# jbrea/BayesianOptimization.jl

Measured on AMD Instinct MI355X. Metric: acquisition-candidates/sec (N=3000,d=8), higher is better.
Workload: dtype f64

## Files before the change

bayesianoptimization.jl_amd/csrc/bohip.hip:

```cpp
#include "../../include/bohip.h"
#include "../../include/bohip_paths.h"
#include "../../include/bohip_fit.h"
#include "../../include/bohip_qei.h"
#include "../../include/bohip_acq.h"
#include "kernels_linalg.hip"
#include "kernels_chol.hip"
#include "kernels_exec.hip"
#include "kernels_score.hip"
#include "kernels_batch.hip"
#include "kernels_sample.hip"
#include "kernels_qei.hip"
#include "kernels_path.hip"
#include "kernels_ascent.hip"
#include "kernels_fit.hip"
#include "kernels_small.hip"
#include "direct_l.h"

#include <algorithm>
#include <atomic>
#include <chrono>
#include <cerrno>
#include <cmath>
#include <cstdio>
#include <cstring>
// ... 36 lines not shown
struct bohip_gp {
    int device = 0, d = 0, kern = 0;
    int64_t n = 0, cap = 0, ld = 0;
    double *dX = nullptr, *dy = nullptr, *dL = nullptr, *dW = nullptr, *dWT = nullptr, *dS = nullptr;
    double *dalpha = nullptr, *dr = nullptr, *dt = nullptr, *dmll = nullptr;
    double* dApp = nullptr;
    int* dinfo = nullptr;
    unsigned* dchol_flags = nullptr;
    double* dchol_idl = nullptr;
    std::vector<double> hX, hy;
    double loglen[DMAX], logsig = 0.0, lognoise = -2.0, beta = 0.0;
    bool stale = true;
    int64_t n_factored = 0;
    hipStream_t stream = nullptr, own_stream = nullptr;
    hipStream_t side_stream = nullptr;
    hipEvent_t ev_panels = nullptr, ev_bulk = nullptr;
    hipStream_t col_stream = nullptr;
    hipEvent_t ev_inv = nullptr;
    hipEvent_t ev_gate = nullptr;
    ExTask* dex_tasks = nullptr;
    size_t ex_cap = 0;
    bool ex_bulk4_ok = false;
    int ex_T = 0, ex_nsf = 0, ex_inv_g = -1, ex_grp_min = -1, ex_qbeg[EX_NQ + 1] = {0};
    bool w_done = false;
    double* dKsT = nullptr;
    unsigned long long* dclk = nullptr;
    int* dpieces = nullptr;
    std::vector<int> hpieces;
    int n_pieces = 0, pieces_T = -1;
    int64_t pieces_cap = 0;
    int64_t pieces_alpha = -1;
    int64_t kst_rows = 0;
    int64_t chunk_now = 0;
    int64_t score_launches = 0;
    double *dVT = nullptr, *dUT = nullptr;
    int64_t vt_rows = 0;
    double *dq = nullptr, *dmu_raw = nullptr, *dXs = nullptr, *dmu = nullptr, *dvar = nullptr, *dscore = nullptr;
    int64_t q_cap = 0, r_cap = 0, xs_cap = 0;
    Best *dblock_best = nullptr, *dbest = nullptr;
    int64_t bb_cap = 0;
    unsigned* dfz_cnt = nullptr;
    Best* dfz_best = nullptr;
    int64_t fz_cap = 0;
    bool fz_dirty = false;
    char* dpr = nullptr;
    size_t pr_bytes = 0;
    std::vector<int> hpr_pieces;
    int* pr_pieces_at = nullptr;
    unsigned* hprune_stat = nullptr;
    unsigned prune_seen = 0;
    bool prune_retry = false;
    int prune_r2_form = -1;
    int prune_skip = 0;
    double* dBV = nullptr;
    int64_t bv_rows = 0, bv_ld = 0;
    char* dbatch = nullptr;
    size_t batch_bytes = 0;
    double* dgrad = nullptr;
    double asc_ftol_abs = 0.0, asc_xtol_rel = 0.0, asc_stopval = INFINITY;
    double asc_maxtime = 0.0;
    int64_t batch_hint = 0;
    double* dsplit = nullptr;
    int64_t split_cap = 0;
    const SmallFold* asc_fold = nullptr;
    bool asc_fold_done = false;
    const unsigned* asc_go = nullptr;
    double* dgparts = nullptr;
    unsigned* dgcount = nullptr;
    double* dsm = nullptr;
    size_t sm_bytes = 0;
    unsigned* dsm_cnt = nullptr;
    int sm_cnt_T = 0;
    double* hpin = nullptr;
    double* dschur = nullptr;
    AscentState asc{};
    double* asc_block = nullptr;
    int* asc_ints = nullptr;
    double* asc_hio = nullptr;
    double* asc_dio = nullptr;
    size_t asc_io_cap = 0;
    int* asc_hints = nullptr;
    double* asc_bounds = nullptr;
    Best* asc_best = nullptr;
    int64_t asc_cap = 0;
    int64_t grad_cap = 0;
    Best* dthompson = nullptr;
    double* ddmll_parts = nullptr;
    double* fit_ws = nullptr;
    char* fit_io = nullptr;
    size_t fit_ws_bytes = 0, fit_io_bytes = 0;
    double *dVV = nullptr, *dcov = nullptr;
    int64_t cov_cap = 0;
    double *sjL = nullptr, *sjS = nullptr, *sjW = nullptr, *sjWT = nullptr, *sjF = nullptr, *sj_scal = nullptr;
    int* sj_info = nullptr;
    Best* sj_part = nullptr;
    int64_t sj_cap = 0;
    size_t sjF_cap = 0, sj_part_cap = 0;
    char* qei_ws = nullptr;
    size_t qei_bytes = 0;
    int64_t dmll_cap = 0;
    int64_t thompson_cap = 0;
    void* comm = nullptr;
    int comm_rank = 0, comm_n = 0;
    int64_t comm_exchanges = 0;
    Best *csend = nullptr, *crecv = nullptr, *cfinal = nullptr;
    int64_t crec_cap = 0;
// ... 122 lines not shown
    {
        const size_t Tm = (size_t)(g->ld / TILE) + 1;
        HIPCHK(hipMalloc(&g->dchol_flags, chol_flag_words((int)std::min<size_t>(Tm, CHOL_DF_TCAP)) * sizeof(unsigned)));
        HIPCHK(hipMalloc(&g->dchol_idl, Tm * CH_PANELS * 256 * 8));
    }
    HIPCHK(hipMemsetAsync(g->dL, 0, mat, g->stream));
    HIPCHK(hipMemsetAsync(g->dW, 0, mat, g->stream));
    HIPCHK(hipMemsetAsync(g->dWT, 0, mat, g->stream));
    HIPCHK(hipMemsetAsync(g->dS, 0, mat, g->stream));
    if (g->n > 0) {
        HIPCHK(hipMemcpyAsync(g->dX, g->hX.data(), (size_t)g->n * g->d * 8, hipMemcpyHostToDevice, g->stream));
        HIPCHK(hipMemcpyAsync(g->dy, g->hy.data(), (size_t)g->n * 8, hipMemcpyHostToDevice, g->stream));
    }
    g->stale = true;
    return 0;
}

static int g_bulk_pieces = 4;
static int g_sample_mfma_min = 200;
static int g_path_mfma_min = 24;
static int g_split = 1;
static int g_asc_wg_nmax = 256;
static const double g_asc_first_step = 0.1;
static int g_asc_fold = 1;
static int g_asc_lockstep = 0;
static int g_small_mfma = 1;
static int g_small_m = 0;
static int g_small_r = -1;
static int g_inv_hi_h = 16;
static int g_chol_df = 1;
static bool g_chol_df_strict = false;
static bool g_chol_df_dump = false;
static int g_chol_df_tmax = 96;
static std::atomic<int> g_chol_df_skip{0}, g_chol_df_backoff{0};
static unsigned long long g_chol_spin_ticks = CH_SPIN_TICKS_DEFAULT;
static int g_chol_exec_patience_us = 1000;
static int g_chol_exec_fill_inv = 1;
static int g_chol_exec_inv_pairs = 0;
static std::atomic<int> g_chol_inv_grp_min{28};
static std::atomic<int> g_chol_inv_g{8};
static int g_chol_nsf = 3;
static int g_chol_exec_urgent = -1;
static int g_chol_exec_second = 1;
static int g_small_zero_copy = 1;
static int g_chol_exec_nbu = 2;
static int g_chol_exec_fast = -1;
static int g_chol_exec_pairs = -1;
static int g_chol_exec_wgs = -1;
static int g_append_alpha_inc = 1;
static int g_fuse_finish = 1;
static int64_t g_chunk_rows_forced = 0;
static int g_halve_lo = -1, g_halve_hi = -1;
static int g_prune_m = -1;
static int g_ks8 = 1;
static int launch_gemm_nt(bohip_gp* g, const GemmNTParams& p, int batch = 1, hipStream_t st = nullptr, bool hi = false) {
    if (p.mt <= 0 || p.nt64 <= 0 || p.kc <= 0 || batch <= 0) return 0;
    if (hi) hipLaunchKernelGGL(k_gemm_nt_hi, dim3(p.mt * p.nt64, batch), dim3(GEMM_THREADS_8), glds3_lds_bytes<4>(), st ? st : g->stream, p);
    else hipLaunchKernelGGL(k_gemm_nt, dim3(p.mt * p.nt64, batch), dim3(GEMM_THREADS_8), glds3_lds_bytes<4>(), st ? st : g->stream, p);
    HIPCHK(hipGetLastError());
    return 0;
}

static int device_cus();
static void read_dev_knobs() {
#if BOHIP_DEV_KNOBS
    struct Knob { const char* name; int* v; int lo, hi; };
    static int chunk_rows = 0, dump = 0;
    const Knob knobs[] = {
        {"BOHIP_CHOL_DF_TMAX", &g_chol_df_tmax, 0, CHOL_DF_TCAP}, {"BOHIP_INV_HI_H", &g_inv_hi_h, 0, 1 << 20},
        {"BOHIP_CHOL_EXEC_PAIRS", &g_chol_exec_pairs, -1, 64},
        {"BOHIP_CHOL_EXEC_URGENT", &g_chol_exec_urgent, 1, 1 << 20}, {"BOHIP_CHOL_NSF", &g_chol_nsf, 1, CH_NSF_MAX},
        {"BOHIP_CHOL_EXEC_PATIENCE_US", &g_chol_exec_patience_us, 0, 1 << 30}, {"BOHIP_CHOL_EXEC_FILL_INV", &g_chol_exec_fill_inv, 0, 1},
        {"BOHIP_CHOL_EXEC_INV_PAIRS", &g_chol_exec_inv_pairs, 0, 1}, {"BOHIP_CHOL_EXEC_WGS", &g_chol_exec_wgs, 1, 1 << 20}, {"BOHIP_KS8", &g_ks8, 0, 1},
        {"BOHIP_CHOL_EXEC_FAST", &g_chol_exec_fast, -1, 1 << 20},
        {"BOHIP_CHOL_EXEC_SECOND", &g_chol_exec_second, 0, 1}, {"BOHIP_SMALL_ZERO_COPY", &g_small_zero_copy, 0, 1}, {"BOHIP_CHOL_EXEC_NBU", &g_chol_exec_nbu, 0, 16}, {"BOHIP_CHUNK_ROWS", &chunk_rows, 0, 1 << 30},
        {"BOHIP_TRIGEMM_HALVE_LO", &g_halve_lo, 0, 1 << 20}, {"BOHIP_TRIGEMM_HALVE_HI", &g_halve_hi, 0, 1 << 20}, {"BOHIP_FUSE_FINISH", &g_fuse_finish, 0, 1}, {"BOHIP_PRUNE_M", &g_prune_m, -1, 1 << 16},
        {"BOHIP_APPEND_ALPHA_INC", &g_append_alpha_inc, 0, 1}, {"BOHIP_BULK_PIECES", &g_bulk_pieces, 0, 8}, {"BOHIP_SPLIT", &g_split, 0, 1},
        {"BOHIP_SMALL_R", &g_small_r, 0, SMALL_MAX}, {"BOHIP_SMALL_M", &g_small_m, 0, 1 << 20}, {"BOHIP_CHOL_DF_DUMP", &dump, 0, 1},
    };
    for (const Knob& k : knobs)
        if (const char* e = getenv(k.name)) *k.v = std::min(k.hi, std::max(k.lo, atoi(e)));
    g_chunk_rows_forced = chunk_rows;
    g_chol_df_dump = dump != 0;
#endif
}

static int one_time_kernel_setup() {
    static bool done_dev[64] = {false};
    int dev = 0;
    HIPCHK(hipGetDevice(&dev));
    bool& done = done_dev[dev & 63];
    if (done) return 0;
    HIPCHK(hipFuncSetAttribute((const void*)k_potf2_inv, hipFuncAttributeMaxDynamicSharedMemorySize, POTF2_LDS_BYTES));
    HIPCHK(hipFuncSetAttribute((const void*)k_gemm_nt, hipFuncAttributeMaxDynamicSharedMemorySize, glds3_lds_bytes<4>()));
    HIPCHK(hipFuncSetAttribute((const void*)k_trigemm_sq<1>, hipFuncAttributeMaxDynamicSharedMemorySize, glds3_lds_bytes<4>()));
    HIPCHK(hipFuncSetAttribute((const void*)k_trigemm_sq<2>, hipFuncAttributeMaxDynamicSharedMemorySize, glds3_lds_bytes<4>()));
    HIPCHK(hipFuncSetAttribute((const void*)k_trigemm_rows, hipFuncAttributeMaxDynamicSharedMemorySize, RS_LDS_BYTES));
    HIPCHK(hipFuncSetAttribute((const void*)k_batch_cond<true>, hipFuncAttributeMaxDynamicSharedMemorySize, BATCH_LDS_MAX));
    HIPCHK(hipFuncSetAttribute((const void*)k_batch_cond<false>, hipFuncAttributeMaxDynamicSharedMemorySize, BATCH_LDS_MAX));
    HIPCHK(hipFuncSetAttribute((const void*)k_chol_chain, hipFuncAttributeMaxDynamicSharedMemorySize, CH_LDS_BYTES));
    HIPCHK(hipFuncSetAttribute((const void*)k_gemm_nt_hi, hipFuncAttributeMaxDynamicSharedMemorySize, glds3_lds_bytes<4>()));
    HIPCHK(hipFuncSetAttribute((const void*)k_chol_exec, hipFuncAttributeMaxDynamicSharedMemorySize, glds3_lds_bytes<4>()));
    HIPCHK(hipFuncSetAttribute((const void*)k_trimv_stream<TRIMV_D>, hipFuncAttributeMaxDynamicSharedMemorySize, trimv_lds_bytes(TRIMV_D)));
    HIPCHK(hipFuncSetAttribute((const void*)k_path_mfma<true>, hipFuncAttributeMaxDynamicSharedMemorySize, (int)path_mfma_lds_bytes(DMAX)));
    HIPCHK(hipFuncSetAttribute((const void*)k_path_mfma<false>, hipFuncAttributeMaxDynamicSharedMemorySize, (int)path_mfma_lds_bytes(DMAX)));
    if (const char* e = getenv("BOHIP_CHOL_DATAFLOW")) g_chol_df = atoi(e);
    if (const char* e = getenv("BOHIP_CHOL_SPIN_US")) g_chol_spin_ticks = 100ull * (unsigned long long)std::max(1, atoi(e));
    if (const char* e = getenv("BOHIP_CHOL_INV_G")) g_chol_inv_g = std::min(64, std::max(0, atoi(e)));
    if (const char* e = getenv("BOHIP_CHOL_INV_GRP_MIN")) g_chol_inv_grp_min = std::max(0, atoi(e));
    if (const char* e = getenv("BOHIP_ASC_WG_NMAX")) g_asc_wg_nmax = std::max(0, atoi(e));
    if (const char* e = getenv("BOHIP_ASC_LOCKSTEP")) { g_asc_lockstep = atoi(e) == 1; g_asc_fold = atoi(e) != 2; }
    if (const char* e = getenv("BOHIP_SMALL_MFMA")) g_small_mfma = atoi(e);
    if (const char* e = getenv("BOHIP_SAMPLE_MFMA_MIN")) g_sample_mfma_min = std::max(1, atoi(e));
    g_chol_df_strict = getenv("BOHIP_CHOL_DF_STRICT") != nullptr;
    read_dev_knobs();
    done = true;
    return 0;
}

static int launch_rows_trimv(bohip_gp* g, const double* W, int64_t N0, const double* rows, int P, double* out, int upper);
static int compute_alpha(bohip_gp* g) {
    const int64_t N = g->n;
    g->alpha_inc_run = 0;
    hipLaunchKernelGGL(k_sub_mean, dim3((N + 255) / 256), dim3(256), 0, g->stream, g->dy, g->beta, N, g->dr);
    HIPCHK(hipGetLastError());
    CHK(launch_rows_trimv(g, g->dW, N, g->dr, 1, g->dt, 0));
    CHK(launch_rows_trimv(g, g->dWT, N, g->dt, 1, g->dalpha, 1));
    HIPCHK(hipMemcpyAsync(g->dW + N * g->ld, g->dalpha, (size_t)N * 8, hipMemcpyDeviceToDevice, g->stream));
    return 0;
// ... 845 lines not shown
        HIPCHK(hipMalloc(&g->dq, (size_t)(2 * T * (Rpad + SLACK)) * 8));
        g->q_cap = 2 * T * (Rpad + SLACK);
    }
    if (g->r_cap < Rpad) {
        for (double** p : {&g->dmu_raw, &g->dmu, &g->dvar, &g->dscore})
            if (*p) { hipFree(*p); *p = nullptr; }
        HIPCHK(hipMalloc(&g->dmu_raw, (Rpad + SLACK) * 8));
        HIPCHK(hipMalloc(&g->dmu, Rpad * 8));
        HIPCHK(hipMalloc(&g->dvar, Rpad * 8));
        HIPCHK(hipMalloc(&g->dscore, Rpad * 8));
        g->r_cap = Rpad;
    }
    const int64_t tiles = Rpad / CTILE + 2;
    if (g->fz_cap < tiles) {
        if (g->dfz_cnt) hipFree(g->dfz_cnt);
        if (g->dfz_best) hipFree(g->dfz_best);
        g->dfz_cnt = nullptr; g->dfz_best = nullptr; g->fz_cap = 0;
        HIPCHK(hipMalloc(&g->dfz_cnt, (size_t)(tiles + 1 + 16) * sizeof(unsigned)));
        HIPCHK(hipMalloc(&g->dfz_best, (size_t)tiles * sizeof(Best)));
        HIPCHK(hipMemsetAsync(g->dfz_cnt, 0, (size_t)(tiles + 1 + 16) * sizeof(unsigned), g->stream));
        g->fz_cap = tiles;
    }
    const int64_t nb = (R + 255) / 256 + 1;
    if (g->bb_cap < nb) {
        if (g->dblock_best) hipFree(g->dblock_best);
        g->dblock_best = nullptr;
        HIPCHK(hipMalloc(&g->dblock_best, nb * sizeof(Best)));
        g->bb_cap = nb;
    }
    return 0;
}
static int ensure_grad_scratch(bohip_gp* g) {
    if (g->vt_rows >= g->kst_rows && g->dVT) return 0;
    for (double** p : {&g->dVT, &g->dUT})
        if (*p) { hipFree(*p); *p = nullptr; }
    const size_t bytes = (size_t)g->kst_rows * g->ld * 8;
    HIPCHK(hipMalloc(&g->dVT, bytes));
    HIPCHK(hipMalloc(&g->dUT, bytes));
    HIPCHK(hipMemsetAsync(g->dVT, 0, bytes, g->stream));
    g->vt_rows = g->kst_rows;
    return 0;
}
static int ensure_xs(bohip_gp* g, int64_t R) {
    if (g->xs_cap < R * g->d) {
        if (g->dXs) hipFree(g->dXs);
        g->dXs = nullptr;
        HIPCHK(hipMalloc(&g->dXs, std::max<size_t>(8, (size_t)R * g->d * 8)));
        g->xs_cap = R * g->d;
    }
    return 0;
}

template <int DT>
static void launch_kstar(bohip_gp* g, const double* dXs, int64_t r0, int64_t r1, int64_t Npad, const KernelHyper& hp, const KstarParts* kp) {
    const int rb = r1 - r0 <= 32 && !kp ? 2 : 16;
    dim3 grid((Npad + 255) / 256, (r1 - r0 + rb - 1) / rb);
    if (kp)
        LAUNCH_FAM(fam_low(hp), (k_kstar<DT, true, true>), (k_kstar<DT, false, true>), grid, dim3(256), 0, g->stream, g->dX, g->n, Npad, dXs,
                   r0, r1, hp, g->dKsT, g->ld, rb, *kp);
    else
        LAUNCH_FAM(fam_low(hp), (k_kstar<DT, true>), (k_kstar<DT, false>), grid, dim3(256), 0, g->stream, g->dX, g->n, Npad, dXs, r0, r1, hp,
                   g->dKsT, g->ld, rb, KstarParts{});
}

static void trigemm_pieces(int T, int64_t alpha_row, std::vector<int>& out) {
    int lo = 0, hi = 0;
    if (g_halve_lo >= 0) { lo = std::min(g_halve_lo, T); hi = std::min(std::max(g_halve_hi, lo), T); }
    struct P { double cost; int code; };
    std::vector<P> ps;
    for (int rt = 0; rt < T; ++rt) {
        const int64_t live = alpha_row + 1 - (int64_t)rt * TILE;
        if (live <= TILE / 2) { ps.push_back({(rt + 0.5) / 2.0, rt | PIECE_UPPER_SOLO << 16}); continue; }
        if (rt >= lo && rt < hi) {
            ps.push_back({(rt + 0.5) / 2.0, rt | PIECE_UPPER << 16});
            ps.push_back({(rt + 1.0) / 2.0, rt | PIECE_LOWER << 16});
        } else {
            ps.push_back({rt + 1.0, rt | PIECE_WHOLE << 16});
        }
    }
    std::stable_sort(ps.begin(), ps.end(), [](const P& a, const P& b) { return a.cost > b.cost; });
    out.clear();
    for (const P& q : ps) out.push_back(q.code);
}
static int ensure_pieces(bohip_gp* g, int T, int64_t alpha_row) {
    if (g->pieces_T == T && g->pieces_alpha == alpha_row && g->dpieces) return 0;
    std::vector<int> ps;
    trigemm_pieces(T, alpha_row, ps);
    if (T > 65535) return fail(BOHIP_E_UNSUPPORTED, "too many row tiles");
    if ((int64_t)ps.size() > g->pieces_cap) {
        if (g->dpieces) { HIPCHK(hipStreamSynchronize(g->stream)); HIPCHK(hipFree(g->dpieces)); g->dpieces = nullptr; }
        g->pieces_cap = 2 * (int64_t)ps.size() + 64;
        HIPCHK(hipMalloc(&g->dpieces, (size_t)g->pieces_cap * sizeof(int)));
    }
    g->hpieces = ps;
    HIPCHK(hipMemcpyAsync(g->dpieces, g->hpieces.data(), ps.size() * sizeof(int), hipMemcpyHostToDevice, g->stream));
    g->n_pieces = (int)ps.size();
    g->pieces_T = T; g->pieces_alpha = alpha_row;
    return 0;
}

static int launch_trigemm(bohip_gp* g, int T, int64_t ncand, int64_t N, int64_t Rpad, int64_t r0, double* VT,
                          FuseParams fz = FuseParams{}) {
    const int CT = (int)((ncand + CTILE - 1) / CTILE), n_local = (CT + 7) / 8;
    CHK(ensure_pieces(g, T, N));
    const int NP = g->n_pieces;
    fz.T = T;
    if (g->timing) {
        if (!g->dclk) {
            HIPCHK(hipMalloc(&g->dclk, 2 * sizeof(unsigned long long)));
            HIPCHK(hipMemsetAsync(g->dclk, 0, 2 * sizeof(unsigned long long), g->stream));
        }
        fz.clk = g->dclk;
    }
    if (g_ks8)
        hipLaunchKernelGGL(k_trigemm_sq<2>, dim3(8 * n_local * NP), dim3(GEMM_THREADS_8), glds3_lds_bytes<4>(), g->stream, g->dW,
                           g->ld, g->dKsT, g->ld, g->dpieces, NP, CT, N, g->dq, Rpad, g->dmu_raw, r0, VT, g->ld, fz);
    else
        hipLaunchKernelGGL(k_trigemm_sq<1>, dim3(8 * n_local * NP), dim3(GEMM_THREADS), glds3_lds_bytes<4>(), g->stream, g->dW,
                           g->ld, g->dKsT, g->ld, g->dpieces, NP, CT, N, g->dq, Rpad, g->dmu_raw, r0, VT, g->ld, fz);
    HIPCHK(hipGetLastError());
    return 0;
}

template <int DT>
static void launch_kstar(bohip_gp* g, const double* dXs, int64_t r0, int64_t r1, int64_t Npad, const KernelHyper& hp, const KstarParts* kp);
static int launch_kstar_any(bohip_gp* g, const double* dXs, int64_t r0, int64_t r1, int64_t Npad, const KernelHyper& hp,
                            const KstarParts* kp = nullptr) {
    if (g->d <= 2) launch_kstar<2>(g, dXs, r0, r1, Npad, hp, kp);
    else if (g->d <= 4) launch_kstar<4>(g, dXs, r0, r1, Npad, hp, kp);
    else if (g->d <= 8) launch_kstar<8>(g, dXs, r0, r1, Npad, hp, kp);
    else if (g->d <= 16) launch_kstar<16>(g, dXs, r0, r1, Npad, hp, kp);
    else if (g->d <= 32) launch_kstar<32>(g, dXs, r0, r1, Npad, hp, kp);
    else launch_kstar<64>(g, dXs, r0, r1, Npad, hp, kp);
    HIPCHK(hipGetLastError());
    return 0;
}

static int ensure_small_counters(bohip_gp* g) {
    if (g->dgparts) return 0;
    HIPCHK(hipMalloc(&g->dgparts, (size_t)SMALL_MAX * 16 * (2 * DMAX + 2) * 8));
    HIPCHK(hipMalloc(&g->dgcount, (SMALL_MAX + 1) * sizeof(unsigned)));
    HIPCHK(hipMemsetAsync(g->dgcount, 0, (SMALL_MAX + 1) * sizeof(unsigned), g->stream));
    return 0;
}
static bool split_applicable(const bohip_gp* g);
static int64_t small_limit(const bohip_gp* g) {
    if (g_small_r >= 0) return g_small_r;
    if (split_applicable(g)) return std::min<int64_t>(SMALL_MAX, std::max<int64_t>(16, (20 + 260000 / std::max<int64_t>(g->n, 1)) / 16 * 16));
    return std::min<int64_t>(SMALL_MAX, 90 + 300000 / std::max<int64_t>(g->n, 1));
}
static int64_t path_R(const bohip_gp* g, int64_t R) { return std::max(R, g->batch_hint); }
#ifdef BOHIP_SMALL_TRACE
static unsigned long long* g_small_trace = nullptr;
extern "C" int bohip_debug_small_trace_read(unsigned long long* out) {
    if (!g_small_trace) return -1;
    return hipMemcpy(out, g_small_trace, 8192 * 16 * 8, hipMemcpyDeviceToHost) == hipSuccess ? 0 : -2;
}
#endif
template <int DT, int G>
static void launch_small_pass(bohip_gp* g, const SmallCommon& sc, const SmallCommon& scu, const SmallV& sv, const SmallU* su, const KernelHyper& hp,
                              int npass) {
    const bool lo = fam_low(hp);
    LAUNCH_FAM(lo, (k_small_v<DT, G, true>), (k_small_v<DT, G, false>), dim3((unsigned)sc.ntiles, (unsigned)npass), dim3(SP_THREADS), 0,
               g->stream, sc, sv, hp);
    if (su) {
        if (DT == 64 && su->sv.ap.acq == ACQ_LOGEI)
            LAUNCH_FAM(lo, (k_small_u_logei64<true>), (k_small_u_logei64<false>), dim3((unsigned)sc.ntiles, (unsigned)npass), dim3(SP_THREADS), 0,
                       g->stream, scu, *su, hp);
        else
            LAUNCH_FAM(lo, (k_small_u<DT, G, true>), (k_small_u<DT, G, false>), dim3((unsigned)sc.ntiles, (unsigned)npass), dim3(SP_THREADS), 0,
                       g->stream, scu, *su, hp);
    }
}
template <int DT>
static void launch_small_pass_g(bohip_gp* g, int G, const SmallCommon& sc, const SmallCommon& scu, const SmallV& sv, const SmallU* su,
                                const KernelHyper& hp, int npass) {
    if constexpr (DT <= 16) {
        if (G == 1) return launch_small_pass<DT, 1>(g, sc, scu, sv, su, hp, npass);
        if (G == 2) return launch_small_pass<DT, 2>(g, sc, scu, sv, su, hp, npass);
        if (G == 3) return launch_small_pass<DT, 3>(g, sc, scu, sv, su, hp, npass);
    }
    launch_small_pass<DT, 4>(g, sc, scu, sv, su, hp, npass);
}
static int small_pass_mfma(bohip_gp* g, const double* dXs, int64_t R, const AcqParams& ap, double* d_mu, double* d_var, double* d_score,
                           Best* d_best, int64_t best_off, double* d_grad) {
    const int N = (int)g->n, T = (N + TILE - 1) / TILE, P = (int)R, npass = (P + 15) / 16, DTm = g->d <= 2 ? 2 : g->d <= 4 ? 4 : g->d <= 8 ? 8 : g->d <= 16 ? 16 : g->d <= 32 ? 32 : 64;
// ... 228 lines not shown
    HIPCHK(hipGetLastError());
    return 0;
}
static int pruned_pass(bohip_gp* g, const double* dXs, int64_t R, int m, const AcqParams& ap, Best* d_best, int64_t best_off,
                       double* ub_host = nullptr, bool long_form = false) {
    CHK(one_time_kernel_setup());
    if (!g->hprune_stat) {
        HIPCHK(hipHostMalloc((void**)&g->hprune_stat, 64, hipHostMallocDefault));
        g->hprune_stat[0] = 0u;
    }
    const int64_t N = g->n, Npad = round_up(N + 1, TILE), Rpad = round_up(R, TILE) + TILE, ld = g->ld;
    const int T = (int)(Npad / TILE);
    const int64_t P = Npad / 64;
    CHK(ensure_pieces(g, T, N));
    std::vector<int> pa, pb;
    for (int c : g->hpieces) ((c & 0xffff) < m ? pa : pb).push_back(c);
    auto al = [](size_t b) { return (b + 255) / 256 * 256; };
    const size_t o_ks = 0, o_q2 = o_ks + al((size_t)Rpad * ld * 8), o_mu2 = o_q2 + al((size_t)2 * T * Rpad * 8),
                 o_ub = o_mu2 + al((size_t)Rpad * 8), o_l1 = o_ub + al((size_t)Rpad * 8), o_l2 = o_l1 + al((size_t)PRUNE_K1 * 4),
                 o_mark = o_l2 + al((size_t)Rpad * 4), o_cnt = o_mark + al((size_t)Rpad * 4), o_rec = o_cnt + 256,
                 o_parts = o_rec + 256, o_pc = o_parts + al((size_t)2 * P * Rpad * 8), total = o_pc + al((3 * g->hpieces.size() + 8) * 4);
    bool fresh = false;
    if (g->pr_bytes < total) {
        fresh = true;
        if (g->dpr) { HIPCHK(hipStreamSynchronize(g->stream)); HIPCHK(hipFree(g->dpr)); g->dpr = nullptr; g->pr_bytes = 0; }
        HIPCHK(hipMalloc(&g->dpr, total));
        g->pr_bytes = total;
    }
    char* b = g->dpr;
    double *ks2 = (double*)(b + o_ks), *q2 = (double*)(b + o_q2), *mu2 = (double*)(b + o_mu2), *ub = (double*)(b + o_ub);
    int *l1 = (int*)(b + o_l1), *l2 = (int*)(b + o_l2), *mark = (int*)(b + o_mark), *pcs = (int*)(b + o_pc);
    const KstarParts kp{g->dW + N * ld, (double*)(b + o_parts), Rpad};
    unsigned* cnt = (unsigned*)(b + o_cnt);
    Best* rec = (Best*)(b + o_rec);
    const std::vector<int> hv = rows_halves(g->hpieces);
    const int nh = rows_halves_from(hv, m);
    std::vector<int> both = pa;
    both.insert(both.end(), pb.begin(), pb.end());
    both.insert(both.end(), hv.begin(), hv.end());
    if (fresh || g->hpr_pieces != both || g->pr_pieces_at != pcs) {
        g->pr_pieces_at = pcs;
        g->hpr_pieces = both;
        HIPCHK(hipMemcpyAsync(pcs, g->hpr_pieces.data(), both.size() * sizeof(int), hipMemcpyHostToDevice, g->stream));
    }
    if (g->timing && !g->dclk) {
        HIPCHK(hipMalloc(&g->dclk, 2 * sizeof(unsigned long long)));
        HIPCHK(hipMemsetAsync(g->dclk, 0, 2 * sizeof(unsigned long long), g->stream));
    }
    g->q_tiles = T;
    g->score_launches = 1;
    const KernelHyper hp = make_hyper(g);
    const double sigma2 = std::exp(2.0 * g->logsig);
    const int k1 = (int)std::min<int64_t>(PRUNE_K1, R);
    t_begin(g, "kstar");
    CHK(launch_kstar_any(g, dXs, 0, R, Npad, hp, &kp));
    t_end(g);
    t_begin(g, "trigemm_sq");
    FuseParams fz{};
    fz.T = T;
    CHK(launch_trigemm_on(g, g->dKsT, pcs, (int)pa.size(), (int)((R + CTILE - 1) / CTILE), g->dq, Rpad, g->dmu_raw, fz));
    PruneBound bd{};
    bd.parts = kp.parts; bd.P = P; bd.ldp = Rpad; bd.Npad = Npad; bd.q = g->dq; bd.ldq = Rpad; bd.R = R; bd.m = m;
    bd.sigma2 = sigma2; bd.beta = g->beta; bd.ap = ap; bd.ub = ub;
    hipLaunchKernelGGL(k_prune_bound, dim3((unsigned)((R + 63) / 64)), dim3(64), 0, g->stream, bd);
    if (ub_host) {
        t_end(g);
        HIPCHK(hipGetLastError());
        HIPCHK(hipMemcpyAsync(ub_host, ub, (size_t)R * 8, hipMemcpyDeviceToHost, g->stream));
        HIPCHK(hipStreamSynchronize(g->stream));
        return 0;
    }
    static_assert(PRUNE_R_MAX <= (int64_t)SELECT_THREADS * SELECT_PER, "k_prune_select holds the whole batch in one workgroup");
    hipLaunchKernelGGL(k_prune_select, dim3(1), dim3(SELECT_THREADS), 0, g->stream, (const double*)ub, R, k1, l1, mark, cnt, rec);
    HIPCHK(hipGetLastError());
    PruneFinish pf{};
    pf.q = g->dq; pf.ldq = Rpad; pf.q2 = q2; pf.ldq2 = Rpad; pf.mu2 = mu2; pf.m = m; pf.T = T; pf.sigma2 = sigma2; pf.beta = g->beta;
    pf.ap = ap; pf.rec = rec;
    const int* hvd = pcs + pa.size() + pb.size();
    pf.ub = ub; pf.mark = mark; pf.R = R; pf.cnt2 = cnt + 1; pf.best_off = (long long)best_off;
    if (nh > 0) {
        pf.list = l1; pf.cnt = cnt; pf.list2 = l2; pf.best_out = d_best; pf.stat = g->hprune_stat;
        CHK(launch_trigemm_rows(g, g->dKsT, hvd, nh, l1, cnt, k1, q2, Rpad, mu2, 0, &pf, cnt + PRUNE_ARRIVE));
        const int64_t cap = R - k1;
        pf.list = l2; pf.cnt = cnt + 1; pf.list2 = nullptr;
        if (cap > 0 && !long_form) {
            CHK(launch_trigemm_rows(g, g->dKsT, hvd, nh, l2, cnt + 1, INT_MAX, q2, Rpad, mu2, PRUNE_R2_GROUPS, &pf, cnt + PRUNE_ARRIVE + 1));
        } else if (cap > 0) {
            if (cap > PRUNE_ROWS_CAP) {
                hipLaunchKernelGGL(k_prune_gather, dim3((unsigned)cap), dim3(256), 0, g->stream, (const int*)l2, (const unsigned*)(cnt + 1),
                                   (const double*)g->dKsT, ld, Npad, ks2, PRUNE_ROWS_CAP, cnt + 2);
                fz.live = cnt + 2;
                CHK(launch_trigemm_on(g, ks2, pcs + pa.size(), (int)pb.size(), (int)((cap + CTILE - 1) / CTILE), q2, Rpad, mu2, fz));
            }
            CHK(launch_trigemm_rows(g, g->dKsT, hvd, nh, l2, cnt + 1, (int)std::min<int64_t>(cap, PRUNE_ROWS_CAP), q2, Rpad, mu2));
            hipLaunchKernelGGL(k_prune_finish, dim3(1), dim3(256), 0, g->stream, pf);
            HIPCHK(hipGetLastError());
        }
        t_end(g);
        return 0;
    }
    for (int round = 0; round < 2; ++round) {
        const int* list = round == 0 ? l1 : l2;
        const unsigned* c = cnt + round;
        const int64_t cap = round == 0 ? k1 : R - k1;
        if (cap > 0) {
            hipLaunchKernelGGL(k_prune_gather, dim3((unsigned)cap), dim3(256), 0, g->stream, list, c, (const double*)g->dKsT, ld, Npad, ks2,
                               -1, cnt + 2);
            fz.live = cnt + 2;
            CHK(launch_trigemm_on(g, ks2, pcs + pa.size(), (int)pb.size(), (int)((cap + CTILE - 1) / CTILE), q2, Rpad, mu2, fz));
        }
        pf.list = list; pf.cnt = c;
        pf.best_out = round == 1 ? d_best : nullptr;
        pf.stat = round == 1 ? g->hprune_stat : nullptr;
// ... 159 lines not shown
        t_end(g);
        t_begin(g, "gemm_U");
        GemmNTParams p{};
        p.A = g->dVT; p.lda = g->ld; p.B = g->dWT; p.ldb = g->ld; p.C = g->dUT; p.ldc = g->ld;
        p.mt = CT; p.nt64 = 2 * T; p.kc = T * (TILE / KC); p.alpha = 1.0; p.beta = 0.0; p.klo_from_n = 1;
        CHK(launch_gemm_nt(g, p));
        t_end(g);
        t_begin(g, "score+grad");
        const int nb = (int)((r1 - r0 + 255) / 256);
        hipLaunchKernelGGL(k_score, dim3(nb), dim3(256), 0, g->stream, g->dq + r0, Rpad, T, g->dmu_raw + r0, r1 - r0,
                           std::exp(2.0 * g->logsig), g->beta, ap, g->dmu + r0, g->dvar + r0, d_score + r0, (Best*)nullptr);
        CHK(launch_grad_any(g, dXs, r0, r1, hp, ap, d_grad, g->dUT));
        t_end(g);
    }
    return 0;
}

extern "C" {

const char* bohip_last_error(void) { return g_err.c_str(); }
const char* bohip_version(void) { return "bohip 0.1 (gfx950, fp64 mfma 4x4x4)"; }
int bohip_device_count(void) {
    int n = 0;
    if (hipGetDeviceCount(&n) != hipSuccess) return 0;
    return n;
}

int bohip_gp_create(int64_t d, int64_t capacity, int kernel_id, int device, bohip_gp** out) {
    if (!out) return fail(BOHIP_E_ARG, "out is null");
    *out = nullptr;
    if (d < 1 || d > DMAX) return fail(BOHIP_E_ARG, "d must be in [1, 64]");
    if (capacity < 1) capacity = 1;
    if (kernel_id < 0 || kernel_id >= KERN_COUNT) return fail(BOHIP_E_ARG, "unknown kernel_id");
    int ndev = 0;
    if (hipGetDeviceCount(&ndev) != hipSuccess || ndev == 0)
        return fail(BOHIP_E_NODEVICE, "no HIP device visible; libbohip has no CPU fallback");
    if (device < 0 || device >= ndev) return fail(BOHIP_E_ARG, "device ordinal out of range");
    HIPCHK(hipSetDevice(device));
    bohip_gp* g = new bohip_gp();
    g->device = device;
    g->d = (int)d;
    g->kern = kernel_id;
    for (int k = 0; k < DMAX; ++k) g->loglen[k] = 0.0;
    int prio_lo = 0, prio_hi = 0;
    hipDeviceGetStreamPriorityRange(&prio_lo, &prio_hi);
    hipError_t e = hipStreamCreateWithPriority(&g->own_stream, hipStreamNonBlocking, prio_hi);
    if (e == hipSuccess) e = hipStreamCreateWithPriority(&g->side_stream, hipStreamNonBlocking, prio_lo);
    if (e == hipSuccess) e = hipEventCreateWithFlags(&g->ev_panels, hipEventDisableTiming);
    if (e == hipSuccess) e = hipEventCreateWithFlags(&g->ev_bulk, hipEventDisableTiming);
    if (e == hipSuccess) e = hipStreamCreateWithPriority(&g->col_stream, hipStreamNonBlocking, prio_hi);
    if (e == hipSuccess) e = hipEventCreateWithFlags(&g->ev_inv, hipEventDisableTiming);
    if (e == hipSuccess) e = hipEventCreateWithFlags(&g->ev_gate, hipEventDisableTiming);
    if (e != hipSuccess) { delete g; return fail(BOHIP_E_HIP, hipGetErrorString(e)); }
    g->stream = g->own_stream;
    if (hipHostMalloc((void**)&g->hpin, (size_t)(3 * SMALL_R + 2 + 2 * SMALL_R * DMAX) * 8, hipHostMallocDefault) != hipSuccess) g->hpin = nullptr;
    if (hipMalloc(&g->dinfo, sizeof(int)) != hipSuccess || hipMalloc(&g->dmll, 8 * (DMAX + 4)) != hipSuccess ||
        hipMalloc(&g->dbest, 4096 * sizeof(Best)) != hipSuccess) {
        delete g;
        return fail(BOHIP_E_HIP, "hipMalloc failed");
    }
    int rc = alloc_model(g, capacity);
    if (rc != 0) { bohip_gp_destroy(g); return rc; }
    if (const char* e = getenv("BOHIP_JITTER")) {
        double rel = 0.0;
        int tries = 10;
        if (sscanf(e, "%lf,%d", &rel, &tries) >= 1 && rel > 0.0) { g->jitter_rel = rel; g->jitter_tries = std::min(32, std::max(1, tries)); }
    }
    *out = g;
    return 0;
}

int bohip_gp_comm_destroy(bohip_gp* g);
void bohip_gp_destroy(bohip_gp* g) {
    if (!g) return;
    hipSetDevice(g->device);
    if (g->own_stream) hipStreamSynchronize(g->own_stream);
    if (g->comm) bohip_gp_comm_destroy(g);
    free_model(g);
    for (double** p : {&g->dKsT, &g->dq, &g->dmu_raw, &g->dXs, &g->dmu, &g->dvar, &g->dscore, &g->dmll, &g->dVT, &g->dUT})
        if (*p) hipFree(*p);
    if (g->dex_tasks) hipFree(g->dex_tasks);
    if (g->dblock_best) hipFree(g->dblock_best);
    if (g->dbest) hipFree(g->dbest);
    if (g->dfz_cnt) hipFree(g->dfz_cnt);
    if (g->dfz_best) hipFree(g->dfz_best);
    if (g->dpr) hipFree(g->dpr);
    if (g->hprune_stat) hipHostFree(g->hprune_stat);
    if (g->dpieces) hipFree(g->dpieces);
    if (g->dclk) hipFree(g->dclk);
    if (g->dgrad) hipFree(g->dgrad);
    if (g->dBV) hipFree(g->dBV);
    if (g->dbatch) hipFree(g->dbatch);
    if (g->dgparts) hipFree(g->dgparts);
    if (g->dsplit) hipFree(g->dsplit);
    if (g->dgcount) hipFree(g->dgcount);
    if (g->dsm) hipFree(g->dsm);
    if (g->dsm_cnt) hipFree(g->dsm_cnt);
    if (g->hpin) hipHostFree(g->hpin);
    if (g->dschur) hipFree(g->dschur);
    if (g->asc_block) hipFree(g->asc_block);
    if (g->asc_ints) hipFree(g->asc_ints);
    if (g->asc_hints) hipHostFree(g->asc_hints);
    if (g->asc_hio) hipHostFree(g->asc_hio);
    if (g->asc_dio) hipFree(g->asc_dio);
    if (g->asc_bounds) hipFree(g->asc_bounds);
    if (g->asc_best) hipFree(g->asc_best);
    if (g->dthompson) hipFree(g->dthompson);
    if (g->ddmll_parts) hipFree(g->ddmll_parts);
    if (g->fit_ws) hipFree(g->fit_ws);
    if (g->fit_io) hipFree(g->fit_io);
    if (g->dVV) hipFree(g->dVV);
    if (g->dcov) hipFree(g->dcov);
    for (double** p : {&g->sjL, &g->sjS, &g->sjW, &g->sjWT, &g->sjF, &g->sj_scal})
        if (*p) hipFree(*p);
    if (g->sj_info) hipFree(g->sj_info);
    if (g->sj_part) hipFree(g->sj_part);
    if (g->qei_ws) hipFree(g->qei_ws);
    if (g->dinfo) hipFree(g->dinfo);
    for (auto& e : g->tpool) { hipEventDestroy(e.first); hipEventDestroy(e.second); }
    if (g->side_stream) { hipStreamSynchronize(g->side_stream); hipStreamDestroy(g->side_stream); }
    if (g->ev_panels) hipEventDestroy(g->ev_panels);
    if (g->ev_bulk) hipEventDestroy(g->ev_bulk);
    if (g->col_stream) { hipStreamSynchronize(g->col_stream); hipStreamDestroy(g->col_stream); }
    if (g->ev_inv) hipEventDestroy(g->ev_inv);
    if (g->ev_gate) hipEventDestroy(g->ev_gate);
    if (g->own_stream) hipStreamDestroy(g->own_stream);
    delete g;
}

int bohip_gp_set_hyper(bohip_gp* g, const double* loglen, double logsig, double lognoise, double mean_const) {
    if (!g || !loglen) return fail(BOHIP_E_ARG, "null argument");
    const int nl = kern_iso(g->kern) ? 1 : g->d;
    for (int k = 0; k < nl; ++k) g->loglen[k] = loglen[k];
    if (kern_iso(g->kern))
        for (int k = 1; k < g->d; ++k) g->loglen[k] = loglen[0];
    g->logsig = logsig;
    g->lognoise = lognoise;
    g->beta = mean_const;
    g->stale = true;
    return 0;
}

int bohip_gp_append(bohip_gp* g, const double* X, const double* y, int64_t p) {
    if (!g || p < 0 || (p > 0 && (!X || !y))) return fail(BOHIP_E_ARG, "bad arguments");
    HIPCHK(hipSetDevice(g->device));
    t_reset(g);
    int rc = 0;
    bool done = false;
    if (p > 0) {
        const int64_t n_old = g->n, n_new = g->n + p;
        if (n_new > g->cap) {
            g->hX.insert(g->hX.end(), X, X + p * g->d);
            g->hy.insert(g->hy.end(), y, y + p);
            g->n = n_new;
            const int arc = alloc_model(g, std::max<int64_t>(2 * g->cap, n_new));
            if (arc != 0) {
                g->hX.resize((size_t)n_old * g->d);
                g->hy.resize((size_t)n_old);
                g->n = n_old;
                free_model(g);
                g->cap = 0;
                g->stale = true;
                return arc;
            }
        } else {
            const bool staged = g->hpin && p <= SMALL_R && (size_t)p * g->d <= (size_t)SMALL_R * DMAX;
            int* pinfo = nullptr;
            if (staged) {
                double* sx = g->hpin + 3 * SMALL_R + 2;
                double* sy = g->hpin;
                std::memcpy(sx, X, (size_t)p * g->d * 8);
                std::memcpy(sy, y, (size_t)p * 8);
                HIPCHK(hipMemcpyAsync(g->dX + n_old * g->d, sx, (size_t)p * g->d * 8, hipMemcpyHostToDevice, g->stream));
                HIPCHK(hipMemcpyAsync(g->dy + n_old, sy, (size_t)p * 8, hipMemcpyHostToDevice, g->stream));
                pinfo = reinterpret_cast<int*>(g->hpin + 3 * SMALL_R);
                *pinfo = 0;
            } else {
                HIPCHK(hipMemcpyAsync(g->dX + n_old * g->d, X, (size_t)p * g->d * 8, hipMemcpyHostToDevice, g->stream));
// ... 1589 lines not shown
    CHK(ensure_xs(g, R));
    CHK(ensure_score_scratch(g, R));
    if (R > g->chunk_now) return fail(BOHIP_E_UNSUPPORTED, "more than one K*' chunk");
    CHK(one_time_kernel_setup());
    const int64_t N = g->n, Npad = round_up(N + 1, TILE), Rpad = round_up(R, TILE);
    const int T = (int)(Npad / TILE);
    CHK(ensure_pieces(g, T, N));
    const std::vector<int> hv = rows_halves(g->hpieces);
    if (path != 0 && hv.empty()) return fail(BOHIP_E_UNSUPPORTED, "row pieces k_trigemm_rows does not reproduce");
    HIPCHK(hipMemcpyAsync(g->dXs, Xs, (size_t)R * g->d * 8, hipMemcpyHostToDevice, g->stream));
    CHK(launch_kstar_any(g, g->dXs, 0, R, Npad, make_hyper(g)));
    std::vector<double> q((size_t)2 * T * Rpad), mu((size_t)Rpad);
    if (path == 0) {
        CHK(launch_trigemm_on(g, g->dKsT, g->dpieces, g->n_pieces, (int)((R + CTILE - 1) / CTILE), g->dq, Rpad, g->dmu_raw, FuseParams{}));
        HIPCHK(hipMemcpyAsync(q.data(), g->dq, q.size() * 8, hipMemcpyDeviceToHost, g->stream));
        HIPCHK(hipMemcpyAsync(mu.data(), g->dmu_raw, mu.size() * 8, hipMemcpyDeviceToHost, g->stream));
        HIPCHK(hipStreamSynchronize(g->stream));
        for (int t = 0; t < 2 * T; ++t) std::memcpy(q_out + (size_t)t * R, q.data() + (size_t)t * Rpad, (size_t)R * 8);
        std::memcpy(mu_out, mu.data(), (size_t)R * 8);
        return 0;
    }
    std::vector<int> list((size_t)R);
    for (int64_t i = 0; i < R; ++i) list[i] = (int)(R - 1 - i);
    const unsigned n = (unsigned)R;
    char* d = nullptr;
    const size_t o_q = 0, o_mu = o_q + q.size() * 8, o_l = o_mu + mu.size() * 8, o_h = o_l + list.size() * 4, o_c = o_h + hv.size() * 4;
    HIPCHK(hipMalloc(&d, o_c + 16));
    int rc = 0;
    hipMemcpyAsync(d + o_l, list.data(), list.size() * 4, hipMemcpyHostToDevice, g->stream);
    hipMemcpyAsync(d + o_h, hv.data(), hv.size() * 4, hipMemcpyHostToDevice, g->stream);
    hipMemcpyAsync(d + o_c, &n, 4, hipMemcpyHostToDevice, g->stream);
    rc = launch_trigemm_rows(g, g->dKsT, (const int*)(d + o_h), (int)hv.size(), (const int*)(d + o_l), (const unsigned*)(d + o_c), (int)R,
                             (double*)(d + o_q), Rpad, (double*)(d + o_mu), path == 2 ? 1 : 0);
    hipMemcpyAsync(q.data(), d + o_q, q.size() * 8, hipMemcpyDeviceToHost, g->stream);
    hipMemcpyAsync(mu.data(), d + o_mu, mu.size() * 8, hipMemcpyDeviceToHost, g->stream);
    const hipError_t e = hipStreamSynchronize(g->stream);
    hipFree(d);
    if (rc != 0) return rc;
    if (e != hipSuccess) return fail(BOHIP_E_HIP, hipGetErrorString(e));
    for (int t = 0; t < 2 * T; ++t)
        for (int64_t i = 0; i < R; ++i) q_out[(size_t)t * R + list[i]] = q[(size_t)t * Rpad + i];
    for (int64_t i = 0; i < R; ++i) mu_out[list[i]] = mu[i];
    return 0;
}
int64_t bohip_debug_prune_stat(bohip_gp* g) {
    if (!g || !g->hprune_stat) return -1;
    return (int64_t)__atomic_load_n(g->hprune_stat, __ATOMIC_RELAXED);
}
int bohip_debug_prune_round2_form(bohip_gp* g, int form) {
    if (!g || form < -1 || form > 1) return fail(BOHIP_E_ARG, "bad arguments");
    g->prune_r2_form = form;
    return 0;
}
int bohip_debug_set_chol_inv_g(int g_new) {
    return g_chol_inv_g.exchange(std::min(64, std::max(0, g_new)));
}
int bohip_debug_exec_throughput(bohip_gp* g, unsigned qmask, int hot, int wgs, double* ms_out, double* gflop_out) {
    if (!g || !ms_out || g->n == 0) return BOHIP_E_ARG;
    hipSetDevice(g->device);
    CHK(one_time_kernel_setup());
    const int T = (int)(round_up(g->n + 1, TILE) / TILE);
    if (T <= 3) return BOHIP_E_UNSUPPORTED;
    std::vector<ExTask> all, run;
    int qb[EX_NQ + 1], qb2[EX_NQ + 1];
    exec_task_list(g->dL, g->dS, g->dW, g->dWT, g->dchol_flags, g->ld, T, g_chol_nsf, g_chol_inv_g, all, qb);
    double fl = 0.0;
    qb2[0] = 0;
    for (int qi = 0; qi < EX_NQ; ++qi) {
        if ((qmask >> qi) & 1u)
            for (int i = qb[qi]; i < qb[qi + 1]; ++i) {
                ExTask t = all[i];
                for (int d = 0; d < EX_NDEP; ++d) { t.dep_idx[d] = EX_NONE; t.dep_want[d] = 0; }
                t.sig_idx[0] = t.sig_idx[1] = EX_NONE;
                t.kc_split = 0; t.dep2_idx[0] = t.dep2_idx[1] = EX_NONE;
                if (hot && (qi == EX_QBULK || qi == EX_QWAVE)) { t.A = g->dS; t.B = g->dS + (int64_t)TILE * g->ld; }
                fl += 2.0 * TILE * CTILE * KC * t.kc;
                run.push_back(t);
            }
        qb2[qi + 1] = (int)run.size();
    }
    if (run.empty()) return BOHIP_E_ARG;
    ExTask* dt = nullptr;
    HIPCHK(hipMalloc(&dt, run.size() * sizeof(ExTask)));
    HIPCHK(hipMemcpy(dt, run.data(), run.size() * sizeof(ExTask), hipMemcpyHostToDevice));
    HIPCHK(hipMemsetAsync(g->dchol_flags, 0, chol_flag_words(T) * sizeof(unsigned), g->stream));
    ExQueues q{};
    q.tasks = dt;
    for (int i = 0; i <= EX_NQ; ++i) q.qbeg[i] = qb2[i];
    q.flags = g->dchol_flags;
    q.abort = g->dchol_flags + chol_abort_word(T);
    q.heads = q.abort + 1;
    q.ld = g->ld;
    q.spin_ticks = g_chol_spin_ticks;
    const int exec_wgs = wgs > 0 ? wgs : std::max(2, std::min(g_chol_exec_wgs > 0 ? g_chol_exec_wgs : 1 << 20, 2 * std::max(1, device_cus() - (9 + g_chol_nsf + 6))));
    q.nurgent = std::max(1, std::min(exec_wgs / 8, g_chol_exec_urgent > 0 ? g_chol_exec_urgent : (T >= 56 ? 16 : 32)));
    const int pairs_ = g_chol_exec_pairs == 0 ? 0 : 1;
        q.stride[0] = 1; q.stride[1] = 1; q.stride[2] = pairs_ ? 2 : 1; q.stride[EX_QBULK] = pairs_ >= 2 ? 2 * std::min(pairs_, 4) : (pairs_ ? 2 : 1);
    q.stride[EX_QROWS] = q.stride[EX_QWAVE] = g_chol_exec_inv_pairs ? 2 : 1;
    q.fill_inv = g_chol_exec_fill_inv;
    q.patience_ticks = (unsigned)g_chol_exec_patience_us * 100u;
    hipEvent_t e0, e1;
    HIPCHK(hipEventCreate(&e0)); HIPCHK(hipEventCreate(&e1));
    HIPCHK(hipEventRecord(e0, g->stream));
    hipLaunchKernelGGL(k_chol_exec, dim3(exec_wgs), dim3(GEMM_THREADS_8), glds3_lds_bytes<4>(), g->stream, q);
    HIPCHK(hipGetLastError());
    HIPCHK(hipEventRecord(e1, g->stream));
// ... 29 lines not shown
```

bayesianoptimization.jl_amd/csrc/kernels_score.hip:

```cpp
#include "gemm_core.h"
#include "acq_log.h"

namespace bohip {

template <bool LOW>
__device__ __forceinline__ double cov_from_r_fast(int fam, double sigma2, double r) {
    if constexpr (LOW) {
        return matern_lo_k(fam, sigma2, r);
    } else {
        if (fam == FAM_M52) {
            const double R = sqrt(r), s = sqrt(5.0) * R;
            return sigma2 * (1.0 + s + 5.0 / 3.0 * r) * exp(-s);
        }
        return sigma2 * exp(-0.5 * r);
    }
}

struct KstarParts {
    const double* alpha;
    double* parts;
    int64_t ldp;
};
__device__ __forceinline__ void swap32(double a, double b, double& x, double& y) {
    const unsigned long long ua = (unsigned long long)__double_as_longlong(a), ub = (unsigned long long)__double_as_longlong(b);
    const auto lo = __builtin_amdgcn_permlane32_swap((unsigned)ua, (unsigned)ub, false, false);
    const auto hi = __builtin_amdgcn_permlane32_swap((unsigned)(ua >> 32), (unsigned)(ub >> 32), false, false);
    x = __longlong_as_double((long long)((unsigned long long)hi[0] << 32 | lo[0]));
    y = __longlong_as_double((long long)((unsigned long long)hi[1] << 32 | lo[1]));
}
template <int BIT>
__device__ __forceinline__ double halve_sum(double a, double b, int lane) {
    const bool up = lane & BIT;
    return (up ? b : a) + __shfl_xor(up ? a : b, BIT);
}
__device__ __forceinline__ void group_sum4(const double* p, int lane, double& sm, double& sa) {
    double x0, y0, x1, y1;
    swap32(p[0], p[2], x0, y0);
    swap32(p[1], p[3], x1, y1);
    sm = halve_sum<16>(x0 + y0, x1 + y1, lane);
    sa = halve_sum<16>(fabs(x0) + fabs(y0), fabs(x1) + fabs(y1), lane);
}
__device__ __forceinline__ double wave_finish(double s) {
    s += __shfl_xor(s, 2);
    s += __shfl_xor(s, 1);
    return s;
}

template <int DT, bool LOW, bool PARTS = false>
__global__ __launch_bounds__(256) void k_kstar(const double* __restrict__ X, int64_t N, int64_t Npad,
                                               const double* __restrict__ Xs, int64_t r_begin, int64_t r_end,
                                               KernelHyper hp, double* __restrict__ KsT, int64_t ldk, int rb, KstarParts kp) {
    __shared__ double xs_l[16 * DT];
    const int d = hp.d;
    const int64_t j = blockIdx.x * 256 + threadIdx.x;
    const int64_t r0 = r_begin + (int64_t)blockIdx.y * rb;
    const int64_t r1 = min(r0 + rb, r_end);
    for (int t = threadIdx.x; t < rb * DT; t += 256) {
        const int64_t r = r0 + t / DT;
        const int k = t % DT;
        xs_l[t] = (r < r1 && k < d) ? Xs[r * d + k] : 0.0;
    }
    double xj[DT], w[DT];
#pragma unroll
    for (int k = 0; k < DT; ++k) {
        xj[k] = (k < d && j < N) ? X[j * d + k] : 0.0;
        w[k] = k < d ? hp.il2[k] : 0.0;
    }
    __syncthreads();
    if (j >= Npad) return;
    const int nc = (int)(r1 - r0);
    if constexpr (PARTS) {
        const double aj = kp.alpha[j];
        const int lane = threadIdx.x & 63;
        double um[2], ua[2], tm0 = 0.0, ta0 = 0.0;
#pragma unroll
        for (int g = 0; g < 4; ++g) {
            double p[4];
#pragma unroll
            for (int i = 0; i < 4; ++i) {
                const int c = 4 * g + i;
                p[i] = 0.0;
                if (c < nc) {
                    double rr = 0.0;
#pragma unroll
                    for (int k = 0; k < DT; ++k) {
                        const double t = xj[k] - xs_l[c * DT + k];
                        rr += w[k] * (t * t);
                    }
                    const double v = (j < N) ? cov_from_r_fast<LOW>(hp.fam, hp.sigma2, rr) : 0.0;
                    KsT[(r0 + c - r_begin) * ldk + j] = v;
                    p[i] = aj * v;
                }
            }
            double tm, ta;
            group_sum4(p, lane, tm, ta);
            if (g & 1) {
                um[g >> 1] = halve_sum<8>(tm0, tm, lane);
                ua[g >> 1] = halve_sum<8>(ta0, ta, lane);
            } else {
                tm0 = tm;
                ta0 = ta;
            }
            __builtin_amdgcn_sched_barrier(0);
        }
        const double sm = wave_finish(halve_sum<4>(um[0], um[1], lane)), sa = wave_finish(halve_sum<4>(ua[0], ua[1], lane));
        const int c = 8 * ((lane >> 2) & 1) + 4 * ((lane >> 3) & 1) + 2 * (lane >> 5) + ((lane >> 4) & 1);
        if ((lane & 3) < 2 && c < nc) {
// ... 1170 lines not shown
```

Baseline: 25.97 million.

## Split pruned-pass kstar into head and tail, overlapping tail with trigemm on a side stream

The kstar kernel in the pruned scoring pass is split by column blocks. The head blocks the trigemm needs run on the main stream, and the remaining tail blocks (which produce only the alpha parts used by the later bound) run on a secondary stream forked and joined with events. The aim is to overlap the tail kstar work with the triangular GEMM instead of serialising them. This adds event record and wait overhead plus possible contention between the concurrent kernels, and it keeps several fork-timing modes behind a knob.

Result: slower. 25.38 million (-2.3%).

```diff
diff --git a/bayesianoptimization.jl_amd/csrc/bohip.hip b/bayesianoptimization.jl_amd/csrc/bohip.hip
--- a/bayesianoptimization.jl_amd/csrc/bohip.hip
+++ b/bayesianoptimization.jl_amd/csrc/bohip.hip
@@ -112,6 +112,8 @@
     bool prune_retry = false;
     int prune_r2_form = -1;
     int prune_skip = 0;
+    hipEvent_t ev_fork = nullptr, ev_join = nullptr;
+    int prune_overlap = -1;
     double* dBV = nullptr;
     int64_t bv_rows = 0, bv_ld = 0;
     char* dbatch = nullptr;
@@ -340,6 +342,7 @@
 static int64_t g_chunk_rows_forced = 0;
 static int g_halve_lo = -1, g_halve_hi = -1;
 static int g_prune_m = -1;
+static int g_prune_overlap = 1;
 static int g_ks8 = 1;
 static int launch_gemm_nt(bohip_gp* g, const GemmNTParams& p, int batch = 1, hipStream_t st = nullptr, bool hi = false) {
     if (p.mt <= 0 || p.nt64 <= 0 || p.kc <= 0 || batch <= 0) return 0;
@@ -363,6 +366,7 @@
         {"BOHIP_CHOL_EXEC_FAST", &g_chol_exec_fast, -1, 1 << 20},
         {"BOHIP_CHOL_EXEC_SECOND", &g_chol_exec_second, 0, 1}, {"BOHIP_SMALL_ZERO_COPY", &g_small_zero_copy, 0, 1}, {"BOHIP_CHOL_EXEC_NBU", &g_chol_exec_nbu, 0, 16}, {"BOHIP_CHUNK_ROWS", &chunk_rows, 0, 1 << 30},
         {"BOHIP_TRIGEMM_HALVE_LO", &g_halve_lo, 0, 1 << 20}, {"BOHIP_TRIGEMM_HALVE_HI", &g_halve_hi, 0, 1 << 20}, {"BOHIP_FUSE_FINISH", &g_fuse_finish, 0, 1}, {"BOHIP_PRUNE_M", &g_prune_m, -1, 1 << 16},
+        {"BOHIP_PRUNE_OVERLAP", &g_prune_overlap, 0, 4},
         {"BOHIP_APPEND_ALPHA_INC", &g_append_alpha_inc, 0, 1}, {"BOHIP_BULK_PIECES", &g_bulk_pieces, 0, 8}, {"BOHIP_SPLIT", &g_split, 0, 1},
         {"BOHIP_SMALL_R", &g_small_r, 0, SMALL_MAX}, {"BOHIP_SMALL_M", &g_small_m, 0, 1 << 20}, {"BOHIP_CHOL_DF_DUMP", &dump, 0, 1},
     };
@@ -1314,15 +1318,19 @@
 }
 
 template <int DT>
-static void launch_kstar(bohip_gp* g, const double* dXs, int64_t r0, int64_t r1, int64_t Npad, const KernelHyper& hp, const KstarParts* kp) {
+static void launch_kstar(bohip_gp* g, const double* dXs, int64_t r0, int64_t r1, int64_t Npad, const KernelHyper& hp, const KstarParts* kp,
+                         int jb0, int jb1, hipStream_t st) {
     const int rb = r1 - r0 <= 32 && !kp ? 2 : 16;
-    dim3 grid((Npad + 255) / 256, (r1 - r0 + rb - 1) / rb);
+    jb0 = std::max(jb0, 0);
+    jb1 = (int)std::min<int64_t>(jb1, (Npad + 255) / 256);
+    if (jb0 >= jb1) return;
+    dim3 grid(jb1 - jb0, (r1 - r0 + rb - 1) / rb);
     if (kp)
-        LAUNCH_FAM(fam_low(hp), (k_kstar<DT, true, true>), (k_kstar<DT, false, true>), grid, dim3(256), 0, g->stream, g->dX, g->n, Npad, dXs,
-                   r0, r1, hp, g->dKsT, g->ld, rb, *kp);
+        LAUNCH_FAM(fam_low(hp), (k_kstar<DT, true, true>), (k_kstar<DT, false, true>), grid, dim3(256), 0, st, g->dX, g->n, Npad, dXs,
+                   r0, r1, hp, g->dKsT, g->ld, rb, *kp, jb0);
     else
-        LAUNCH_FAM(fam_low(hp), (k_kstar<DT, true>), (k_kstar<DT, false>), grid, dim3(256), 0, g->stream, g->dX, g->n, Npad, dXs, r0, r1, hp,
-                   g->dKsT, g->ld, rb, KstarParts{});
+        LAUNCH_FAM(fam_low(hp), (k_kstar<DT, true>), (k_kstar<DT, false>), grid, dim3(256), 0, st, g->dX, g->n, Npad, dXs, r0, r1, hp,
+                   g->dKsT, g->ld, rb, KstarParts{}, jb0);
 }
 
 static void trigemm_pieces(int T, int64_t alpha_row, std::vector<int>& out) {
@@ -1385,15 +1393,17 @@
 }
 
 template <int DT>
-static void launch_kstar(bohip_gp* g, const double* dXs, int64_t r0, int64_t r1, int64_t Npad, const KernelHyper& hp, const KstarParts* kp);
+static void launch_kstar(bohip_gp* g, const double* dXs, int64_t r0, int64_t r1, int64_t Npad, const KernelHyper& hp, const KstarParts* kp,
+                         int jb0, int jb1, hipStream_t st);
 static int launch_kstar_any(bohip_gp* g, const double* dXs, int64_t r0, int64_t r1, int64_t Npad, const KernelHyper& hp,
-                            const KstarParts* kp = nullptr) {
-    if (g->d <= 2) launch_kstar<2>(g, dXs, r0, r1, Npad, hp, kp);
-    else if (g->d <= 4) launch_kstar<4>(g, dXs, r0, r1, Npad, hp, kp);
-    else if (g->d <= 8) launch_kstar<8>(g, dXs, r0, r1, Npad, hp, kp);
-    else if (g->d <= 16) launch_kstar<16>(g, dXs, r0, r1, Npad, hp, kp);
-    else if (g->d <= 32) launch_kstar<32>(g, dXs, r0, r1, Npad, hp, kp);
-    else launch_kstar<64>(g, dXs, r0, r1, Npad, hp, kp);
+                            const KstarParts* kp = nullptr, int jb0 = 0, int jb1 = INT_MAX, hipStream_t st = nullptr) {
+    if (!st) st = g->stream;
+    if (g->d <= 2) launch_kstar<2>(g, dXs, r0, r1, Npad, hp, kp, jb0, jb1, st);
+    else if (g->d <= 4) launch_kstar<4>(g, dXs, r0, r1, Npad, hp, kp, jb0, jb1, st);
+    else if (g->d <= 8) launch_kstar<8>(g, dXs, r0, r1, Npad, hp, kp, jb0, jb1, st);
+    else if (g->d <= 16) launch_kstar<16>(g, dXs, r0, r1, Npad, hp, kp, jb0, jb1, st);
+    else if (g->d <= 32) launch_kstar<32>(g, dXs, r0, r1, Npad, hp, kp, jb0, jb1, st);
+    else launch_kstar<64>(g, dXs, r0, r1, Npad, hp, kp, jb0, jb1, st);
     HIPCHK(hipGetLastError());
     return 0;
 }
@@ -1728,13 +1738,37 @@
     const KernelHyper hp = make_hyper(g);
     const double sigma2 = std::exp(2.0 * g->logsig);
     const int k1 = (int)std::min<int64_t>(PRUNE_K1, R);
+    const int jb_all = (int)((Npad + 255) / 256), jb_head = std::min(jb_all, (TILE * m + 255) / 256);
+    const int ov_mode = g->prune_overlap >= 0 ? g->prune_overlap : g_prune_overlap;
+    const hipStream_t tail_st = ov_mode == 2 || ov_mode == 4 ? g->side_stream : g->col_stream;
+    const bool fork_late = ov_mode >= 3;
+    const bool overlap = ov_mode != 0 && tail_st && g->ev_fork && g->ev_join && jb_head < jb_all;
+    int rc = 0;
+    bool forked = false;
+    auto fork_tail = [&]() -> int {
+        HIPCHK(hipEventRecord(g->ev_fork, g->stream));
+        HIPCHK(hipStreamWaitEvent(tail_st, g->ev_fork, 0));
+        forked = true;
+        return launch_kstar_any(g, dXs, 0, R, Npad, hp, &kp, jb_head, jb_all, tail_st);
+    };
+    if (overlap && !fork_late) rc = fork_tail();
     t_begin(g, "kstar");
-    CHK(launch_kstar_any(g, dXs, 0, R, Npad, hp, &kp));
+    if (rc == 0) rc = launch_kstar_any(g, dXs, 0, R, Npad, hp, &kp, 0, overlap ? jb_head : jb_all);
     t_end(g);
+    if (overlap && fork_late && rc == 0) rc = fork_tail();
     t_begin(g, "trigemm_sq");
     FuseParams fz{};
     fz.T = T;
-    CHK(launch_trigemm_on(g, g->dKsT, pcs, (int)pa.size(), (int)((R + CTILE - 1) / CTILE), g->dq, Rpad, g->dmu_raw, fz));
+    if (rc == 0) rc = launch_trigemm_on(g, g->dKsT, pcs, (int)pa.size(), (int)((R + CTILE - 1) / CTILE), g->dq, Rpad, g->dmu_raw, fz);
+    if (forked) {
+        hipError_t e = hipEventRecord(g->ev_join, tail_st);
+        if (e == hipSuccess) e = hipStreamWaitEvent(g->stream, g->ev_join, 0);
+        if (e != hipSuccess) {
+            hipStreamSynchronize(tail_st);
+            if (rc == 0) rc = fail(BOHIP_E_HIP, std::string("pruned pass, join: ") + hipGetErrorString(e));
+        }
+    }
+    CHK(rc);
     PruneBound bd{};
     bd.parts = kp.parts; bd.P = P; bd.ldp = Rpad; bd.Npad = Npad; bd.q = g->dq; bd.ldq = Rpad; bd.R = R; bd.m = m;
     bd.sigma2 = sigma2; bd.beta = g->beta; bd.ap = ap; bd.ub = ub;
@@ -2000,6 +2034,8 @@
     if (e == hipSuccess) e = hipEventCreateWithFlags(&g->ev_inv, hipEventDisableTiming);
     if (e == hipSuccess) e = hipEventCreateWithFlags(&g->ev_gate, hipEventDisableTiming);
     if (e != hipSuccess) { delete g; return fail(BOHIP_E_HIP, hipGetErrorString(e)); }
+    if (hipEventCreateWithFlags(&g->ev_fork, hipEventDisableTiming) != hipSuccess) g->ev_fork = nullptr;
+    if (hipEventCreateWithFlags(&g->ev_join, hipEventDisableTiming) != hipSuccess) g->ev_join = nullptr;
     g->stream = g->own_stream;
     if (hipHostMalloc((void**)&g->hpin, (size_t)(3 * SMALL_R + 2 + 2 * SMALL_R * DMAX) * 8, hipHostMallocDefault) != hipSuccess) g->hpin = nullptr;
     if (hipMalloc(&g->dinfo, sizeof(int)) != hipSuccess || hipMalloc(&g->dmll, 8 * (DMAX + 4)) != hipSuccess ||
@@ -2072,6 +2108,8 @@
     if (g->col_stream) { hipStreamSynchronize(g->col_stream); hipStreamDestroy(g->col_stream); }
     if (g->ev_inv) hipEventDestroy(g->ev_inv);
     if (g->ev_gate) hipEventDestroy(g->ev_gate);
+    if (g->ev_fork) hipEventDestroy(g->ev_fork);
+    if (g->ev_join) hipEventDestroy(g->ev_join);
     if (g->own_stream) hipStreamDestroy(g->own_stream);
     delete g;
 }
@@ -3767,6 +3805,11 @@
     g->prune_r2_form = form;
     return 0;
 }
+int bohip_debug_prune_overlap(bohip_gp* g, int mode) {
+    if (!g || mode < -1 || mode > 1) return fail(BOHIP_E_ARG, "bad arguments");
+    g->prune_overlap = mode;
+    return 0;
+}
 int bohip_debug_set_chol_inv_g(int g_new) {
     return g_chol_inv_g.exchange(std::min(64, std::max(0, g_new)));
 }
diff --git a/bayesianoptimization.jl_amd/csrc/kernels_score.hip b/bayesianoptimization.jl_amd/csrc/kernels_score.hip
--- a/bayesianoptimization.jl_amd/csrc/kernels_score.hip
+++ b/bayesianoptimization.jl_amd/csrc/kernels_score.hip
@@ -49,10 +49,10 @@
 template <int DT, bool LOW, bool PARTS = false>
 __global__ __launch_bounds__(256) void k_kstar(const double* __restrict__ X, int64_t N, int64_t Npad,
                                                const double* __restrict__ Xs, int64_t r_begin, int64_t r_end,
-                                               KernelHyper hp, double* __restrict__ KsT, int64_t ldk, int rb, KstarParts kp) {
+                                               KernelHyper hp, double* __restrict__ KsT, int64_t ldk, int rb, KstarParts kp, int jb0) {
     __shared__ double xs_l[16 * DT];
     const int d = hp.d;
-    const int64_t j = blockIdx.x * 256 + threadIdx.x;
+    const int64_t j = (int64_t)(blockIdx.x + jb0) * 256 + threadIdx.x;
     const int64_t r0 = r_begin + (int64_t)blockIdx.y * rb;
     const int64_t r1 = min(r0 + rb, r_end);
     for (int t = threadIdx.x; t < rb * DT; t += 256) {
```
